# freshman97/LinTransUNet

Hardware: AMD Instinct MI355X
Metric: 128^3 CT patches/sec (fwd+bwd) (higher is better)
Workload: dtype bf16; 1 GPU; MaskTransUnet train step (fwd + 5-level loss + bwd), 128^3 single-channel patches, 2 per GPU, dropout 0.3, random-init weights; global_batch=2, parallelism=dp1, side_stream_concurrent=True, allreduce=none (1 rank)

## Files before the change

include/ltu_hip.h:

```cpp
#ifndef LTU_HIP_H
#define LTU_HIP_H

#include <stdint.h>

#ifdef __cplusplus
extern "C" {
#endif

typedef void* ltu_stream_t;

enum { LTU_F32 = 0, LTU_BF16 = 1 };
enum { LTU_OK = 0, LTU_E_DTYPE = -1, LTU_E_SHAPE = -2, LTU_E_ALIGN = -3, LTU_E_ARG = -4,
       LTU_E_COMM = -100  };
enum { LTU_ACT_NONE = 0, LTU_ACT_LRELU = 1 };

int ltu_version(void);
int ltu_build_flags(void);
int ltu_config_set(const char* name, int value, int clear);
int ltu_selftest_group_reduce(const float* x, float* sum, float* mx, int n, int G, ltu_stream_t s);
#ifdef LTU_EXPERIMENTS
int ltu_selftest_last_arriver(const float* x, float* part, float* out, unsigned* counter, float* sink, int nwg, int n,
                              int rows_per_chunk, int skew, int mode, ltu_stream_t s);
#endif

// ... 107 lines not shown

int ltu_head_softmax_fwd(const void* z, float* p, long long M, int C, int CP, int dtype, ltu_stream_t s);
int ltu_head_softmax_bwd(const float* dp, const float* p, void* dz, long long M, int C, int CP, int dtype, ltu_stream_t s);
int ltu_final_softmax_fwd(const void* z, float* p, int B, int h, int w, int D, int C, int CP, int dtype, ltu_stream_t s);
int ltu_final_softmax_bwd(const float* dp, const float* p, void* dz, int B, int h, int w, int D, int C, int CP, int dtype,
                          ltu_stream_t s);
int ltu_onehot_argmax(const float* p, float* o, long long M, int C, ltu_stream_t s);

int ltu_gate_fwd(const void* u1, const void* u2, const float* sums1, const float* sums2, const float* psi_w,
                 const float* psi_b, const void* skip, float* a_out, void* out, int B, long long S, int C, int dtype,
                 ltu_stream_t s);
int ltu_gate_bwd(const void* dout, const void* u1, const void* u2, const float* sums1, const float* sums2,
                 const float* psi_w, const void* skip, const float* a_in, void* dskip, float* ds_ws, float* dpsi_w,
                 float* dpsi_b, float* bs1, float* bs2, float* ws, long long ws_floats, void* du1, void* du2, int B, long long S, int C,
                 int dtype, ltu_stream_t s);

int ltu_dwconv_fwd(const void* x, const float* w, const float* bias, void* y, int B, int H, int W, int D, int C, float p,
                   uint64_t seed, const uint64_t* step, int dtype, ltu_stream_t s);
long long ltu_dwconv_bwd_ws_floats(int B, int H, int W, int D, int C, int dtype);
int ltu_dwconv_bwd(const void* dy, const void* dy2, const void* x, const float* w, void* dx, float* dw, float* db, float* ws,
                   long long ws_floats, int B, int H, int W, int D, int C, float p, uint64_t seed, const uint64_t* step, int dtype, ltu_stream_t s);

int ltu_roi_plan_size(int B, int H, int W, int roi_size, long long* n_int, long long* n_float, long long* n_hist);
int ltu_roi_plan(const float* prob, int B, int H, int W, int D, int C, int roi_size, float thr, float* box, int* plan_i,
                 float* plan_f, int* hist, ltu_stream_t s);
int ltu_roi_resample(const void* in, void* out, int* plan_i, float* plan_f, int which, int adjoint, int B, int H, int W,
                     int D, int C, int roi_size, int dtype, ltu_stream_t s);

int ltu_trilinear_up(const void* in, const void* in2, void* out, int adjoint, int B, int H, int W, int D, int C, int sd, int dtype,
                     ltu_stream_t s);
// ... 111 lines not shown
```

lintransunet_amd/_lib.py:

```python
import ctypes
import os
from ctypes import c_float, c_int, c_longlong, c_uint64, c_void_p

_HERE = os.path.dirname(os.path.abspath(__file__))
LIB_PATH = os.path.join(_HERE, os.environ.get('LTU_LIB', 'libltu_hip.so'))

P, I, L, F, U = c_void_p, c_int, c_longlong, c_float, c_uint64


class ReduceJob(ctypes.Structure):
    _fields_ = [('part', c_void_p), ('nsplit', c_int), ('n', c_int), ('k', c_int), ('nseg', c_int),
                ('out', c_void_p * 3), ('outb', c_void_p * 3), ('mode', c_int)]


class WgradJob(ctypes.Structure):
    _fields_ = [('grad', c_void_p), ('a', c_void_p), ('dw', c_void_p * 3), ('db', c_void_p * 3),
                ('ldg', c_int), ('lda', c_int), ('nw', c_int), ('M', c_int), ('N', c_int), ('K', c_int)]


WGRAD_GROUP_MAX = 32
CROP_ORIENT_MAX = 64
BLEND_ITEMS_MAX = 32
U8, I16 = 2, 3

# ... 76 lines not shown
    'ltu_instnorm_stats': [P, P, P, L, I, L, I, I, P],
    'ltu_instnorm_apply': [P, P, P, P, I, L, I, I, F, F, U, P, I, P],
    'ltu_instnorm_fwd': [P, P, P, L, P, P, I, L, I, I, F, F, U, P, I, P],
    'ltu_instnorm_bwd': [P, P, P, P, P, P, P, L, P, I, L, I, I, F, F, U, P, I, P],
    'ltu_layernorm_fwd': [P, P, P, P, P, P, L, I, F, F, U, P, I, P],
    'ltu_layernorm_bwd': [P, P, P, P, P, P, P, P, P, P, L, P, L, I, F, U, P, I, P],
    'ltu_gelu_dropout_fwd': [P, P, L, F, U, P, I, P],
    'ltu_gelu_dropout_bwd': [P, P, P, L, F, U, P, I, P],
    'ltu_head_softmax_fwd': [P, P, L, I, I, I, P],
    'ltu_head_softmax_bwd': [P, P, P, L, I, I, I, P],
    'ltu_final_softmax_fwd': [P, P, I, I, I, I, I, I, I, P],
    'ltu_final_softmax_bwd': [P, P, P, I, I, I, I, I, I, I, P],
    'ltu_onehot_argmax': [P, P, L, I, P],
    'ltu_gate_fwd': [P, P, P, P, P, P, P, P, P, I, L, I, I, P],
    'ltu_gate_bwd': [P, P, P, P, P, P, P, P, P, P, P, P, P, P, P, L, P, P, I, L, I, I, P],
    'ltu_dwconv_fwd': [P, P, P, P, I, I, I, I, I, F, U, P, I, P],
    'ltu_dwconv_bwd_ws_floats': [I, I, I, I, I, I],
    'ltu_dwconv_bwd': [P, P, P, P, P, P, P, P, L, I, I, I, I, I, F, U, P, I, P],
    'ltu_roi_plan_size': [I, I, I, I, P, P, P],
    'ltu_roi_plan': [P, I, I, I, I, I, I, F, P, P, P, P, P],
    'ltu_roi_resample': [P, P, P, P, I, I, I, I, I, I, I, I, I, P],
    'ltu_trilinear_up': [P, P, P, I, I, I, I, I, I, I, I, P],
    'ltu_trilinear_adjoint_ws_elems': [I, I, I, I, I, I],
    'ltu_trilinear_adjoint': [P, P, P, P, L, I, I, I, I, I, I, I, P],
    'ltu_loss_ws_floats': [I, L, I],
    'ltu_loss_fwd': [P, P, P, L, P, P, I, L, I, F, F, P, P, P],
    'ltu_loss_bwd': [P, P, P, P, P, I, L, I, P],
    'ltu_loss_wide_ws_floats': [I, L, I],
    'ltu_loss_wide_fwd': [P, P, P, L, P, P, I, L, I, F, F, P, P, P],
    'ltu_loss_wide_bwd': [P, P, P, P, P, I, L, I, P],
# ... 61 lines not shown
```

lintransunet_amd/csrc/pointwise.hip:

```cpp
#include "common.h"
#include "manyclass.h"

static unsigned sgrid(long long n, int per_block = 256) {
  long long blocks = (n + per_block - 1) / per_block;
  if (blocks > 8192) blocks = 8192;
  if (blocks < 1) blocks = 1;
  return (unsigned)blocks;
}
#define GRID_STRIDE(i, n) \
  for (long long i = (long long)blockIdx.x * blockDim.x + threadIdx.x; i < (n); i += (long long)gridDim.x * blockDim.x)

template <typename T>
__global__ void window_embed_kernel(const float* __restrict__ x, T* __restrict__ y, int B, int H, int W, int D) {
  const int h2 = H / 2, w2 = W / 2;
  const long long n = (long long)B * h2 * w2 * D;
  GRID_STRIDE(i, n) {
    const int d = (int)(i % D);
    long long t = i / D;
    const int w = (int)(t % w2);
    t /= w2;
    const int h = (int)(t % h2);
    const int b = (int)(t / h2);
    const float* xb = x + (((long long)b * H + 2 * h) * W + 2 * w) * D + d;
    float4 v = make_float4(xb[0], xb[D], xb[(long long)W * D], xb[(long long)W * D + D]);
// ... 389 lines not shown
}
extern "C" int ltu_onehot_argmax(const float* p, float* o, long long M, int C, ltu_stream_t s) {
  hipLaunchKernelGGL(onehot_argmax_kernel, dim3(sgrid(M)), dim3(256), 0, (hipStream_t)s, p, o, M, C);
  return ltu_check_launch();
}

#define IN_EPS 1e-5f
__device__ __forceinline__ void in_stat2(const float* sums, float invS, float& mean, float& rstd) {
  const float m1 = sums[1] * invS;
  const float var = fmaxf(sums[2] * invS - m1 * m1, 0.f);
  mean = sums[0] + m1;
  rstd = rsqrtf(var + IN_EPS);
}

template <typename T, int G>
__global__ void gate_fwd_kernel(const T* __restrict__ u1, const T* __restrict__ u2, const float* __restrict__ sums1,
                                const float* __restrict__ sums2, const float* __restrict__ psi_w, const float* __restrict__ psi_b,
                                const T* __restrict__ skip, float* __restrict__ a_out, T* __restrict__ out, int B, long long S) {
  const int C = G * 4;
  const int gl = threadIdx.x % G;
  const long long rows = (long long)B * S;
  const float invS = 1.f / (float)S;
  const float4 pw = *reinterpret_cast<const float4*>(psi_w + gl * 4);
  const float pb = psi_b[0];
  const long long rpb = blockDim.x / G;
  for (long long r0 = (long long)blockIdx.x * rpb; r0 < rows; r0 += (long long)gridDim.x * rpb) {
    const long long row = r0 + threadIdx.x / G;
    const bool ok = row < rows;
    float part = 0.f;
    float4 sk = make_float4(0.f, 0.f, 0.f, 0.f);
    if (ok) {
// ... 8 lines not shown
        in_stat2(sums2 + ((long long)b * C + gl * 4 + k) * 3, invS, m2, r2);
        const float r = fmaxf((f4at(a, k) - m1) * r1 + (f4at(c, k) - m2) * r2, 0.f);
        part += r * f4at(pw, k);
      }
    }
    const float sdot = group_sum<G>(part) + pb;
    const float av = 1.f / (1.f + expf(-sdot));
    if (ok) {
      if (gl == 0) a_out[row] = av;
      Vec4<T>::store(out + row * C + gl * 4, make_float4(sk.x * av, sk.y * av, sk.z * av, sk.w * av));
    }
  }
}

template <typename T, int G>
__global__ void gate_bwd_reduce_kernel(const T* __restrict__ dout, const T* __restrict__ u1, const T* __restrict__ u2,
                                       const float* __restrict__ sums1, const float* __restrict__ sums2,
                                       const float* __restrict__ psi_w, const T* __restrict__ skip, const float* __restrict__ a_in,
                                       T* __restrict__ dskip, float* __restrict__ ds_out, float* __restrict__ dpsi_w,
                                       float* __restrict__ dpsi_b, float* __restrict__ bs1, float* __restrict__ bs2,
                                       float* __restrict__ ws, int B, long long S, int rows_per_block) {
  extern __shared__ float red[];
  const int C = G * 4;
  const int gl = threadIdx.x % G, rg = threadIdx.x / G, nrg = blockDim.x / G;
  const int b = blockIdx.y;
  const float invS = 1.f / (float)S;
  const float4 pw = *reinterpret_cast<const float4*>(psi_w + gl * 4);
  float m1[4], r1[4], m2[4], r2[4];
#pragma unroll
  for (int k = 0; k < 4; ++k) {
// ... 14 lines not shown
    const bool ok = sv < s1;
    const long long row = (long long)b * S + sv;
    float4 g = make_float4(0.f, 0.f, 0.f, 0.f), sk = g, a = g, c = g;
    float av = 0.f;
    if (ok) {
      const long long e = row * C + gl * 4;
      g = Vec4<T>::load(dout + e);
      sk = Vec4<T>::load(skip + e);
      a = Vec4<T>::load(u1 + e);
      c = Vec4<T>::load(u2 + e);
      av = a_in[row];
    }
    const float da = group_sum<G>(g.x * sk.x + g.y * sk.y + g.z * sk.z + g.w * sk.w);
    const float ds = da * av * (1.f - av);
    if (ok) {
      Vec4<T>::store(dskip + row * C + gl * 4, make_float4(g.x * av, g.y * av, g.z * av, g.w * av));
      if (gl == 0) { ds_out[row] = ds; accb += ds; }
#pragma unroll
      for (int k = 0; k < 4; ++k) {
        const float h1 = (f4at(a, k) - m1[k]) * r1[k], h2 = (f4at(c, k) - m2[k]) * r2[k];
        const float r = fmaxf(h1 + h2, 0.f);
        const float dr = r > 0.f ? ds * f4at(pw, k) : 0.f;
        acc[k][0] += ds * r;
        acc[k][1] += dr;
        acc[k][2] += dr * h1;
        acc[k][3] += dr * h2;
      }
    }
  }
#pragma unroll
  for (int k = 0; k < 4; ++k) {
// ... 34 lines not shown
  }
  red[zq][el] = a0 + a1;
  __syncthreads();
  if (zq != 0 || i >= n) return;
  float v = 0.f;
#pragma unroll
  for (int q = 0; q < 32; ++q) v += red[q][el];
  const int c = i / 5, which = i % 5;
  if (which == 0) atomicAdd(dpsi_w + c, v);
  else if (which == 1) { bs1[((long long)b * C + c) * 2] += v; bs2[((long long)b * C + c) * 2] += v; }
  else if (which == 2) bs1[((long long)b * C + c) * 2 + 1] += v;
  else if (which == 3) bs2[((long long)b * C + c) * 2 + 1] += v;
  else if (c == 0) atomicAdd(dpsi_b, v);
}

template <typename T, int G>
__global__ void __launch_bounds__(256) gate_bwd_apply_kernel(const T* __restrict__ u1, const T* __restrict__ u2, const float* __restrict__ sums1,
                                      const float* __restrict__ sums2, const float* __restrict__ psi_w,
                                      const float* __restrict__ ds_in, const float* __restrict__ bs1, const float* __restrict__ bs2,
                                      T* __restrict__ du1, T* __restrict__ du2, int B, long long S) {
  constexpr int C = G * 4;
  const int b = blockIdx.y;
  const int gl = threadIdx.x % G;
  const float invS = 1.f / (float)S;
  const float4 pw = *reinterpret_cast<const float4*>(psi_w + gl * 4);
  float m1[4], r1[4], m2[4], r2[4], a1[4], b1[4], a2[4], b2[4];
#pragma unroll
  for (int k = 0; k < 4; ++k) {
    const long long bc = (long long)b * C + gl * 4 + k;
    in_stat2(sums1 + bc * 3, invS, m1[k], r1[k]);
// ... 23 lines not shown
  do {                                                        \
    if ((C) == 8) { constexpr int G = 2; __VA_ARGS__ }        \
    else if ((C) == 16) { constexpr int G = 4; __VA_ARGS__ }  \
    else if ((C) == 32) { constexpr int G = 8; __VA_ARGS__ }  \
    else if ((C) == 64) { constexpr int G = 16; __VA_ARGS__ } \
    else if ((C) == 128) { constexpr int G = 32; __VA_ARGS__ } \
    else if ((C) == 256) { constexpr int G = 64; __VA_ARGS__ } \
    else return LTU_E_SHAPE;                                  \
  } while (0)

extern "C" int ltu_gate_fwd(const void* u1, const void* u2, const float* sums1, const float* sums2, const float* psi_w,
                            const float* psi_b, const void* skip, float* a_out, void* out, int B, long long S, int C, int dtype,
                            ltu_stream_t s) {
  LTU_DISPATCH_T(dtype, {
    GATE_DISPATCH_G(C, {
      const long long rows = (long long)B * S;
      hipLaunchKernelGGL((gate_fwd_kernel<T, G>), dim3(sgrid(rows, 256 / G)), dim3(256), 0, (hipStream_t)s, (const T*)u1,
                         (const T*)u2, sums1, sums2, psi_w, psi_b, (const T*)skip, a_out, (T*)out, B, S);
    });
  });
  return ltu_check_launch();
}

extern "C" int ltu_gate_bwd(const void* dout, const void* u1, const void* u2, const float* sums1, const float* sums2,
                            const float* psi_w, const void* skip, const float* a_in, void* dskip, float* ds_ws, float* dpsi_w,
                            float* dpsi_b, float* bs1, float* bs2, float* ws, long long ws_floats, void* du1, void* du2, int B, long long S,
                            int C, int dtype, ltu_stream_t s) {
  if (ws != nullptr && ws_floats < ltu_norm_ws_floats()) return LTU_E_ARG;
  LTU_DISPATCH_T(dtype, {
    GATE_DISPATCH_G(C, {
      const int nrg = 256 / G;
      long long cap = (1 << 20) / (C * 5);
      if (cap > 2048) cap = 2048;
      long long want = cap / (B > 0 ? B : 1);
      if (want < 1) want = 1;
      long long rows = (S + want - 1) / want;
      if (rows < nrg) rows = nrg;
      rows = (rows + nrg - 1) / nrg * nrg;
      const size_t lds = (size_t)nrg * C * 5 * sizeof(float);
      hipLaunchKernelGGL((gate_bwd_reduce_kernel<T, G>), dim3(cdiv(S, rows), B), dim3(256), lds, (hipStream_t)s, (const T*)dout,
                         (const T*)u1, (const T*)u2, sums1, sums2, psi_w, (const T*)skip, a_in, (T*)dskip, ds_ws, dpsi_w, dpsi_b,
                         bs1, bs2, ws, B, S, (int)rows);
      if (ws != nullptr)
        hipLaunchKernelGGL(gate_fold_kernel, dim3(cdiv(C * 5, 32), B), dim3(1024), 0, (hipStream_t)s, ws, (int)cdiv(S, rows), C,
                           dpsi_w, dpsi_b, bs1, bs2);
      long long ablocks = (S * G + 255) / 256;
      const long long acap = 4096 / (B > 0 ? B : 1) > 1 ? 4096 / (B > 0 ? B : 1) : 1;
      if (ablocks > acap) ablocks = acap;
      hipLaunchKernelGGL((gate_bwd_apply_kernel<T, G>), dim3((unsigned)ablocks, B), dim3(256), 0, (hipStream_t)s,
                         (const T*)u1, (const T*)u2, sums1, sums2, psi_w, ds_ws, bs1, bs2, (T*)du1, (T*)du2, B, S);
    });
  });
  return ltu_check_launch();
}


#define DWH_VOX 360
#define DWH_PD 11
#define DWH_ROWS (36 * DWH_PD)
#define DWH_RUN 4
template <typename T>
__device__ __forceinline__ uint4 add16(uint4 a, uint4 b);
template <>
__device__ __forceinline__ uint4 add16<float>(uint4 a, uint4 b) {
  return make_uint4(__float_as_uint(__uint_as_float(a.x) + __uint_as_float(b.x)), __float_as_uint(__uint_as_float(a.y) + __uint_as_float(b.y)),
                    __float_as_uint(__uint_as_float(a.z) + __uint_as_float(b.z)), __float_as_uint(__uint_as_float(a.w) + __uint_as_float(b.w)));
}
template <>
// ... 305 lines not shown
```

lintransunet_amd/ops.py:

```python
import contextlib
import ctypes
import threading

import torch

from . import _lib

F32, BF16 = 0, 1
ACT_NONE, ACT_LRELU = 0, 1
LRELU_SLOPE = 0.01
_c_void_p = ctypes.c_void_p


def _dt(t):
    if t.dtype == torch.float32:
        return F32
    if t.dtype == torch.bfloat16:
        return BF16
    raise TypeError(f'unsupported activation dtype {t.dtype}')


def _p(t):
    return 0 if t is None else t.data_ptr()

# ... 1361 lines not shown
class _Gate(torch.autograd.Function):

    @staticmethod
    def forward(ctx, skip, up, wx, bx, wg, bg, pw, pb, px, pg):
        lc = ctx.lc = current()
        _chk(skip, 'skip'); _chk(up, 'up')
        B, C = skip.shape[0], skip.shape[-1]
        Cg = up.shape[-1]
        M = skip.numel() // C
        S = M // B
        dev, dt = skip.device, _dt(skip)
        u1 = torch.empty((M, C), device=dev, dtype=skip.dtype)
        u2 = torch.empty((M, C), device=dev, dtype=skip.dtype)
        wxo = px.w[0] if px is not None else _w_operand(wx, skip.dtype)
        wgo = pg.w[0] if pg is not None else _w_operand(wg, skip.dtype)
        _lib.call('ltu_linear_fwd', _p(skip), C, _ptr_array([wxo]), 1, _ptr_array([bx]), _p(u1), C, M, C, C, 0, dt, _s())
        _lib.call('ltu_linear_fwd', _p(up), Cg, _ptr_array([wgo]), 1, _ptr_array([bg]), _p(u2), C, M, C, Cg, 0, dt, _s())
        s1 = lc.scratch_zeros((B, C, 3), dev)
        s2 = lc.scratch_zeros((B, C, 3), dev)
        _lib.call('ltu_instnorm_stats', _p(u1), _p(s1), _p(lc.norm_ws(dev)), _n(lc.norm_ws(dev)), B, S, C, dt, _s())
        _lib.call('ltu_instnorm_stats', _p(u2), _p(s2), _p(lc.norm_ws(dev)), _n(lc.norm_ws(dev)), B, S, C, dt, _s())
        a = torch.empty(M, device=dev, dtype=torch.float32)
        out = torch.empty_like(skip)
        _lib.call('ltu_gate_fwd', _p(u1), _p(u2), _p(s1), _p(s2), _p(pw), _p(pb), _p(skip), _p(a), _p(out), B, S, C, dt, _s())
        ctx.save_for_backward(skip, up, u1, u2, s1, s2, a)
        ctx.params = (wx, bx, wg, bg, pw, pb)
        ctx.prep = (px, pg)
        return out

    @staticmethod
    def backward(ctx, g):
        lc = ctx.lc
        skip, up, u1, u2, s1, s2, a = ctx.saved_tensors
        wx, bx, wg, bg, pw, pb = ctx.params
        px, pg = ctx.prep
        g = g.contiguous()
        B, C = skip.shape[0], skip.shape[-1]
        Cg = up.shape[-1]
        M = skip.numel() // C
        S = M // B
        dev, dt = skip.device, _dt(skip)
        dskip = torch.empty_like(skip)
        ds = torch.empty(M, device=dev, dtype=torch.float32)
        dpw, fpw = _grad_buf(pw)
        dpb, fpb = _grad_buf(pb)
        bs1 = lc.scratch_zeros((B, C, 2), dev)
        bs2 = lc.scratch_zeros((B, C, 2), dev)
        du1 = torch.empty_like(u1)
        du2 = torch.empty_like(u2)
        _lib.call('ltu_gate_bwd', _p(g), _p(u1), _p(u2), _p(s1), _p(s2), _p(pw), _p(skip), _p(a), _p(dskip), _p(ds), _p(dpw),
                  _p(dpb), _p(bs1), _p(bs2), _p(lc.norm_ws(dev)), _n(lc.norm_ws(dev)), _p(du1), _p(du2), B, S, C, dt, _s())
        wxt = px.wt if px is not None else _w_transposed([wx], C, C, skip.dtype)
        wgt = pg.wt if pg is not None else _w_transposed([wg], C, Cg, skip.dtype)
        dup = torch.empty_like(up)
        _lib.call('ltu_linear_fwd', _p(du1), C, _ptr_array([wxt]), 1, _ptr_array([None]), _p(dskip), C, M, C, C, 1, dt, _s())
        _lib.call('ltu_linear_fwd', _p(du2), C, _ptr_array([wgt]), 1, _ptr_array([None]), _p(dup), Cg, M, Cg, C, 0, dt, _s())
        dwx, f1 = _grad_buf(wx)
        dbx, f2 = _grad_buf(bx)
        dwg, f3 = _grad_buf(wg)
        dbg, f4 = _grad_buf(bg)
        def launch(keep):
            w1, w2 = _wgrad_ws(M, C, C, skip), _wgrad_ws(M, C, Cg, skip)
            keep.extend((w1, w2))
            _lib.call('ltu_linear_wgrad', _p(du1), C, _p(skip), C, _ptr_array([dwx]), _ptr_array([dbx]), 1, M, C, C, _p(w1), _n(w1), 0, dt, _s())
            _lib.call('ltu_linear_wgrad', _p(du2), C, _p(up), Cg, _ptr_array([dwg]), _ptr_array([dbg]), 1, M, C, Cg, _p(w2), _n(w2), 0, dt, _s())
        if f1 and f2 and f3 and f4:
            lc.wq_push(launch, (du1, du2, skip, up), 'gate')
        else:
            launch([])
        return (dskip, dup, _grad_done(wx, dwx, f1), _grad_done(bx, dbx, f2), _grad_done(wg, dwg, f3), _grad_done(bg, dbg, f4),
                _grad_done(pw, dpw, fpw), _grad_done(pb, dpb, fpb), None, None)
# ... 110 lines not shown
```

Baseline: 164.0 patches/s.

## Fuse attention-gate projections with instnorm stats and fuse gate backward data path

Adds a forward kernel that computes both gate 1x1 projections with MFMA and accumulates per-channel shifted instance-norm statistics in the same pass, followed by a small fold kernel. This replaces two linear launches plus two stats passes that reread u1/u2. In backward, the elementwise gate gradient is fused with the transposed-weight matmuls that produce dskip and dup, so du1/du2 are not reread. The fused path only covers bf16 with C of 16 or 32 and adds shifted-sum numerics that differ slightly from the old stats path.

```diff
diff --git a/include/ltu_hip.h b/include/ltu_hip.h
--- a/include/ltu_hip.h
+++ b/include/ltu_hip.h
@@ -145,6 +145,14 @@
                  const float* psi_w, const void* skip, const float* a_in, void* dskip, float* ds_ws, float* dpsi_w,
                  float* dpsi_b, float* bs1, float* bs2, float* ws, long long ws_floats, void* du1, void* du2, int B, long long S, int C,
                  int dtype, ltu_stream_t s);
+int ltu_gate_fused_ok(int B, long long S, int C, int Cg, int dtype);
+int ltu_gate_proj_fwd(const void* skip, const void* up, const void* wx, const float* bx, const void* wg, const float* bg, void* u1,
+                      void* u2, float* sums1, float* sums2, float* parts, long long parts_floats, int B, long long S, int C, int dtype,
+                      ltu_stream_t s);
+int ltu_gate_bwd_fused(const void* dout, const void* u1, const void* u2, const float* sums1, const float* sums2,
+                       const float* psi_w, const void* skip, const float* a_in, const void* wxt, const void* wgt, void* dskip,
+                       void* dup, float* ds_ws, float* dpsi_w, float* dpsi_b, float* bs1, float* bs2, float* parts,
+                       long long parts_floats, void* du1, void* du2, int B, long long S, int C, int dtype, ltu_stream_t s);
 
 int ltu_dwconv_fwd(const void* x, const float* w, const float* bias, void* y, int B, int H, int W, int D, int C, float p,
                    uint64_t seed, const uint64_t* step, int dtype, ltu_stream_t s);
diff --git a/lintransunet_amd/_lib.py b/lintransunet_amd/_lib.py
--- a/lintransunet_amd/_lib.py
+++ b/lintransunet_amd/_lib.py
@@ -114,6 +114,9 @@
     'ltu_onehot_argmax': [P, P, L, I, P],
     'ltu_gate_fwd': [P, P, P, P, P, P, P, P, P, I, L, I, I, P],
     'ltu_gate_bwd': [P, P, P, P, P, P, P, P, P, P, P, P, P, P, P, L, P, P, I, L, I, I, P],
+    'ltu_gate_fused_ok': [I, L, I, I, I],
+    'ltu_gate_proj_fwd': [P, P, P, P, P, P, P, P, P, P, P, L, I, L, I, I, P],
+    'ltu_gate_bwd_fused': [P, P, P, P, P, P, P, P, P, P, P, P, P, P, P, P, P, P, L, P, P, I, L, I, I, P],
     'ltu_dwconv_fwd': [P, P, P, P, I, I, I, I, I, F, U, P, I, P],
     'ltu_dwconv_bwd_ws_floats': [I, I, I, I, I, I],
     'ltu_dwconv_bwd': [P, P, P, P, P, P, P, P, L, I, I, I, I, I, F, U, P, I, P],
diff --git a/lintransunet_amd/csrc/gate_fused.hip b/lintransunet_amd/csrc/gate_fused.hip
--- /dev/null
+++ b/lintransunet_amd/csrc/gate_fused.hip
@@ -0,0 +1,366 @@
+#include "common.h"
+
+#define IN_EPS 1e-5f
+__device__ __forceinline__ float gf_rounded(float x) {
+  asm volatile("" : "+v"(x));
+  return x;
+}
+__device__ __forceinline__ void gf_in_stat2(const float* sums, float invS, float& mean, float& rstd) {
+  const float m1 = gf_rounded(sums[1] * invS);
+  const float var = fmaxf(gf_rounded(sums[2] * invS) - gf_rounded(m1 * m1), 0.f);
+  mean = __builtin_fmaf(invS, sums[1], sums[0]);
+  rstd = rsqrtf(var + IN_EPS);
+}
+
+template <int KS, int NT>
+__device__ __forceinline__ void gf_load_w(const uint16_t* __restrict__ w, int N, int li, int lh, bf16x8 (&wf)[NT][KS]) {
+#pragma unroll
+  for (int j = 0; j < NT; ++j)
+#pragma unroll
+    for (int ks = 0; ks < KS; ++ks) {
+      const int n = j * 32 + li;
+      const uint4 v = *reinterpret_cast<const uint4*>(w + (long long)(n < N ? n : 0) * (16 * KS) + ks * 16 + lh * 8);
+      wf[j][ks] = __builtin_bit_cast(bf16x8, n < N ? v : make_uint4(0u, 0u, 0u, 0u));
+    }
+}
+
+template <int KS>
+__device__ __forceinline__ f32x16 gf_mfma(const bf16x8 (&wf)[KS], const uint4 (&x)[KS]) {
+  f32x16 acc;
+#pragma unroll
+  for (int r = 0; r < 16; ++r) acc[r] = 0.f;
+#pragma unroll
+  for (int ks = 0; ks < KS; ++ks) acc = __builtin_amdgcn_mfma_f32_32x32x16_bf16(wf[ks], __builtin_bit_cast(bf16x8, x[ks]), acc, 0, 0, 0);
+  return acc;
+}
+
+__device__ __forceinline__ uint4 gf_quad_swap(const f32x16& acc, const float4 (&bv)[4], int q) {
+  const int r0 = 2 * q, r1 = 2 * q + 1;
+  float p0x = __uint_as_float(pack_bf16x2(acc[4 * r0] + bv[r0].x, acc[4 * r0 + 1] + bv[r0].y));
+  float p0y = __uint_as_float(pack_bf16x2(acc[4 * r0 + 2] + bv[r0].z, acc[4 * r0 + 3] + bv[r0].w));
+  float p1x = __uint_as_float(pack_bf16x2(acc[4 * r1] + bv[r1].x, acc[4 * r1 + 1] + bv[r1].y));
+  float p1y = __uint_as_float(pack_bf16x2(acc[4 * r1 + 2] + bv[r1].z, acc[4 * r1 + 3] + bv[r1].w));
+  permlane32_swap(p1x, p0x);
+  permlane32_swap(p1y, p0y);
+  return make_uint4(__float_as_uint(p1x), __float_as_uint(p1y), __float_as_uint(p0x), __float_as_uint(p0y));
+}
+
+__device__ __forceinline__ void gf_unpack8(const uint4& v, float (&f)[8]) {
+  const uint32_t w[4] = {v.x, v.y, v.z, v.w};
+#pragma unroll
+  for (int i = 0; i < 4; ++i) { f[2 * i] = __uint_as_float(w[i] << 16); f[2 * i + 1] = __uint_as_float(w[i] & 0xffff0000u); }
+}
+
+struct GateProjArgs {
+  const uint16_t *skip, *up, *wx, *wg;
+  const float *bx, *bg;
+  uint16_t *u1, *u2;
+  float* parts;
+  long long S;
+};
+
+template <int C>
+__global__ void __launch_bounds__(256, 2) gate_proj_stats_kernel(const GateProjArgs a) {
+  constexpr int K1 = C / 16, K2 = C / 8, Q = C / 16;
+  __shared__ float red[4][4 * C];
+  const int lane = threadIdx.x & 63, li = lane & 31, lh = lane >> 5, wid = threadIdx.x >> 6;
+  const int b = blockIdx.y;
+  const long long ntile = a.S / 32, nwave = (long long)gridDim.x * 4;
+  const uint16_t* xs = a.skip + (long long)b * a.S * C;
+  const uint16_t* xu = a.up + (long long)b * a.S * (2 * C);
+  uint16_t* y1 = a.u1 + (long long)b * a.S * C;
+  uint16_t* y2 = a.u2 + (long long)b * a.S * C;
+  bf16x8 w1[1][K1], w2[1][K2];
+  gf_load_w<K1, 1>(a.wx, C, li, lh, w1);
+  gf_load_w<K2, 1>(a.wg, C, li, lh, w2);
+  float4 b1[4], b2[4];
+#pragma unroll
+  for (int rr = 0; rr < 4; ++rr) {
+    const int n = 8 * rr + 4 * lh;
+    b1[rr] = (a.bx != nullptr && n < C) ? *reinterpret_cast<const float4*>(a.bx + n) : make_float4(0.f, 0.f, 0.f, 0.f);
+    b2[rr] = (a.bg != nullptr && n < C) ? *reinterpret_cast<const float4*>(a.bg + n) : make_float4(0.f, 0.f, 0.f, 0.f);
+  }
+  auto fetch = [&](long long tile, uint4 (&s)[K1], uint4 (&u)[K2]) {
+    const long long row = tile * 32 + li;
+    const uint16_t* ps = xs + row * C + lh * 8;
+    const uint16_t* pu = xu + row * (2 * C) + lh * 8;
+#pragma unroll
+    for (int ks = 0; ks < K1; ++ks) s[ks] = *reinterpret_cast<const uint4*>(ps + ks * 16);
+#pragma unroll
+    for (int ks = 0; ks < K2; ++ks) u[ks] = *reinterpret_cast<const uint4*>(pu + ks * 16);
+  };
+  uint4 sc[K1], uc[K2];
+  long long tile = (long long)blockIdx.x * 4 + wid;
+  fetch(0, sc, uc);
+  uint4 sh1[Q], sh2[Q];
+  {
+    const f32x16 acc1 = gf_mfma<K1>(w1[0], sc), acc2 = gf_mfma<K2>(w2[0], uc);
+    if (tile < ntile) fetch(tile, sc, uc);
+#pragma unroll
+    for (int q = 0; q < Q; ++q) {
+      const uint4 v1 = gf_quad_swap(acc1, b1, q), v2 = gf_quad_swap(acc2, b2, q);
+      const uint32_t e1[4] = {v1.x, v1.y, v1.z, v1.w}, e2[4] = {v2.x, v2.y, v2.z, v2.w};
+      uint32_t* o1 = &sh1[q].x;
+      uint32_t* o2 = &sh2[q].x;
+#pragma unroll
+      for (int e = 0; e < 4; ++e) {
+        const uint32_t lo1 = __builtin_amdgcn_readlane(e1[e], 0), hi1 = __builtin_amdgcn_readlane(e1[e], 32);
+        const uint32_t lo2 = __builtin_amdgcn_readlane(e2[e], 0), hi2 = __builtin_amdgcn_readlane(e2[e], 32);
+        o1[e] = lh ? hi1 : lo1;
+        o2[e] = lh ? hi2 : lo2;
+      }
+    }
+  }
+  float s1a[Q][8], s1b[Q][8], s2a[Q][8], s2b[Q][8];
+#pragma unroll
+  for (int q = 0; q < Q; ++q)
+#pragma unroll
+    for (int e = 0; e < 8; ++e) { s1a[q][e] = 0.f; s1b[q][e] = 0.f; s2a[q][e] = 0.f; s2b[q][e] = 0.f; }
+  for (; tile < ntile; tile += nwave) {
+    const f32x16 acc1 = gf_mfma<K1>(w1[0], sc), acc2 = gf_mfma<K2>(w2[0], uc);
+    if (tile + nwave < ntile) fetch(tile + nwave, sc, uc);
+    const long long e0 = (tile * 32 + li) * C + (lh ? 0 : 8);
+#pragma unroll
+    for (int q = 0; q < Q; ++q) {
+      const uint4 v1 = gf_quad_swap(acc1, b1, q), v2 = gf_quad_swap(acc2, b2, q);
+      *reinterpret_cast<uint4*>(y1 + e0 + 16 * q) = v1;
+      *reinterpret_cast<uint4*>(y2 + e0 + 16 * q) = v2;
+      float f1[8], f2[8], h1[8], h2[8];
+      gf_unpack8(v1, f1);
+      gf_unpack8(v2, f2);
+      gf_unpack8(sh1[q], h1);
+      gf_unpack8(sh2[q], h2);
+#pragma unroll
+      for (int e = 0; e < 8; ++e) {
+        const float t1 = f1[e] - h1[e], t2 = f2[e] - h2[e];
+        s1a[q][e] += t1; s1b[q][e] += t1 * t1;
+        s2a[q][e] += t2; s2b[q][e] += t2 * t2;
+      }
+    }
+  }
+#pragma unroll
+  for (int q = 0; q < Q; ++q)
+#pragma unroll
+    for (int e = 0; e < 8; ++e) {
+      const float r1a = group_sum<32>(s1a[q][e]), r1b = group_sum<32>(s1b[q][e]);
+      const float r2a = group_sum<32>(s2a[q][e]), r2b = group_sum<32>(s2b[q][e]);
+      if (li == 0) {
+        const int c = 16 * q + (lh ? 0 : 8) + e;
+        red[wid][2 * c] = r1a; red[wid][2 * c + 1] = r1b;
+        red[wid][2 * C + 2 * c] = r2a; red[wid][2 * C + 2 * c + 1] = r2b;
+      }
+    }
+  __syncthreads();
+  if (threadIdx.x < 4 * C) {
+    const int i = threadIdx.x;
+    a.parts[((long long)b * gridDim.x + blockIdx.x) * (4 * C) + i] = (red[0][i] + red[1][i]) + (red[2][i] + red[3][i]);
+  }
+}
+
+template <int NB>
+__global__ void __launch_bounds__(1024) gate_stats_fold_kernel(const float* __restrict__ parts, int nparts, int C, const uint16_t* __restrict__ u1,
+                                                               const uint16_t* __restrict__ u2, long long S, float* __restrict__ sums1,
+                                                               float* __restrict__ sums2) {
+  __shared__ float red[32][33];
+  const int n = 4 * C;
+  const int el = threadIdx.x & 31, zq = threadIdx.x >> 5;
+  const int i = blockIdx.x * 32 + el, b = blockIdx.y;
+  float acc = 0.f;
+  if (i < n) {
+    const float* p = parts + (long long)b * nparts * n + i;
+    for (int z0 = zq; z0 < nparts; z0 += 32 * NB) {
+      float v[NB];
+#pragma unroll
+      for (int k = 0; k < NB; ++k) {
+        const int z = z0 + 32 * k;
+        v[k] = p[(long long)(z < nparts ? z : z0) * n];
+      }
+      float a0 = 0.f, a1 = 0.f, a2 = 0.f, a3 = 0.f;
+#pragma unroll
+      for (int k = 0; k < NB; ++k) {
+        const float t = z0 + 32 * k < nparts ? v[k] : 0.f;
+        if ((k & 3) == 0) a0 += t; else if ((k & 3) == 1) a1 += t; else if ((k & 3) == 2) a2 += t; else a3 += t;
+      }
+      acc += (a0 + a1) + (a2 + a3);
+    }
+  }
+  red[zq][el] = acc;
+  __syncthreads();
+  if (zq != 0 || i >= n) return;
+  float v = 0.f;
+#pragma unroll
+  for (int q = 0; q < 32; ++q) v += red[q][el];
+  const int t = i >= 2 * C, c = (i - t * 2 * C) >> 1, which = i & 1;
+  float* s = (t ? sums2 : sums1) + ((long long)b * C + c) * 3;
+  s[1 + which] = v;
+  if (which == 0) s[0] = bf16_to_f32((t ? u2 : u1)[(long long)b * S * C + c]);
+}
+
+static long long gate_proj_nparts(int B, long long S, int C, long long cap) {
+  const long long ntile = S / 32;
+  long long np = (ntile + 31) / 32;
+  const long long most = 1024 / B > 1 ? 1024 / B : 1;
+  if (np > most) np = most;
+  const long long fit = cap / ((long long)B * 4 * C);
+  if (np > fit) np = fit;
+  return np;
+}
+
+bool gate_fused_shape_ok(int B, long long S, int C, int Cg, int dtype) {
+  return dtype == LTU_BF16 && (C == 16 || C == 32) && Cg == 2 * C && B >= 1 && B <= 65535 && S >= 32 && S % 32 == 0 &&
+         (long long)B * 4 * C <= ltu_norm_ws_floats();
+}
+
+extern "C" int ltu_gate_fused_ok(int B, long long S, int C, int Cg, int dtype) {
+  return gate_fused_shape_ok(B, S, C, Cg, dtype) && !ltu_knob("LTU_NO_GATE_FUSED", 0) ? 1 : 0;
+}
+
+extern "C" int ltu_gate_proj_fwd(const void* skip, const void* up, const void* wx, const float* bx, const void* wg, const float* bg, void* u1,
+                                 void* u2, float* sums1, float* sums2, float* parts, long long parts_floats, int B, long long S, int C,
+                                 int dtype, ltu_stream_t s) {
+  if (!gate_fused_shape_ok(B, S, C, 2 * C, dtype)) return dtype == LTU_BF16 ? LTU_E_SHAPE : LTU_E_DTYPE;
+  if (parts == nullptr) return LTU_E_ARG;
+  const long long np = gate_proj_nparts(B, S, C, ltu_norm_ws_floats());
+  if (np < 1 || parts_floats < (long long)B * np * 4 * C) return LTU_E_ARG;
+  GateProjArgs a;
+  a.skip = (const uint16_t*)skip; a.up = (const uint16_t*)up; a.wx = (const uint16_t*)wx; a.wg = (const uint16_t*)wg;
+  a.bx = bx; a.bg = bg; a.u1 = (uint16_t*)u1; a.u2 = (uint16_t*)u2; a.parts = parts; a.S = S;
+  const dim3 grid((unsigned)np, B), fgrid(cdiv(4 * C, 32), B);
+  hipStream_t st = (hipStream_t)s;
+  if (C == 16) hipLaunchKernelGGL(gate_proj_stats_kernel<16>, grid, dim3(256), 0, st, a);
+  else hipLaunchKernelGGL(gate_proj_stats_kernel<32>, grid, dim3(256), 0, st, a);
+#define GF_FOLD(NB_) \
+  hipLaunchKernelGGL(gate_stats_fold_kernel<NB_>, fgrid, dim3(1024), 0, st, parts, (int)np, C, a.u1, a.u2, S, sums1, sums2)
+  if (np <= 128) GF_FOLD(4); else if (np <= 256) GF_FOLD(8); else if (np <= 512) GF_FOLD(16); else GF_FOLD(32);
+#undef GF_FOLD
+  return ltu_check_launch();
+}
+
+struct GateBwdArgs {
+  const uint16_t *dout, *u1, *u2, *wxt, *wgt;
+  const float *sums1, *sums2, *bs1, *bs2, *psi_w, *a, *ds;
+  uint16_t *du1, *du2, *dskip, *dup;
+  long long S;
+};
+
+template <int C>
+__global__ void __launch_bounds__(256) gate_bwd_fused_kernel(const GateBwdArgs g) {
+  constexpr int KS = C / 16, NT2 = C / 16, Q = C / 16;
+  __shared__ __attribute__((aligned(16))) float cst[9][C];
+  const int lane = threadIdx.x & 63, li = lane & 31, lh = lane >> 5, wid = threadIdx.x >> 6;
+  const int b = blockIdx.y;
+  const float invS = 1.f / (float)g.S;
+  if (threadIdx.x < C) {
+    const int c = threadIdx.x;
+    const long long bc = (long long)b * C + c;
+    float m1, r1, m2, r2;
+    gf_in_stat2(g.sums1 + bc * 3, invS, m1, r1);
+    gf_in_stat2(g.sums2 + bc * 3, invS, m2, r2);
+    cst[0][c] = m1; cst[1][c] = r1; cst[2][c] = m2; cst[3][c] = r2;
+    cst[4][c] = g.bs1[bc * 2] * invS; cst[5][c] = g.bs1[bc * 2 + 1] * invS;
+    cst[6][c] = g.bs2[bc * 2] * invS; cst[7][c] = g.bs2[bc * 2 + 1] * invS;
+    cst[8][c] = g.psi_w[c];
+  }
+  bf16x8 wx[1][KS], wg[NT2][KS];
+  gf_load_w<KS, 1>(g.wxt, C, li, lh, wx);
+  gf_load_w<KS, NT2>(g.wgt, 2 * C, li, lh, wg);
+  __syncthreads();
+  const long long ntile = g.S / 32, nwave = (long long)gridDim.x * 4;
+  const long long base = (long long)b * g.S;
+  struct Tile {
+    uint4 x1[KS], x2[KS], go[Q];
+    float av, ds;
+  };
+  auto fetch = [&](long long tile, Tile& t) {
+    const long long row = base + tile * 32 + li;
+    const long long e = row * C + lh * 8, eo = row * C + (lh ? 0 : 8);
+#pragma unroll
+    for (int ks = 0; ks < KS; ++ks) {
+      t.x1[ks] = *reinterpret_cast<const uint4*>(g.u1 + e + ks * 16);
+      t.x2[ks] = *reinterpret_cast<const uint4*>(g.u2 + e + ks * 16);
+    }
+#pragma unroll
+    for (int q = 0; q < Q; ++q) t.go[q] = *reinterpret_cast<const uint4*>(g.dout + eo + q * 16);
+    t.av = g.a[row];
+    t.ds = g.ds[row];
+  };
+  const float4 zero4[4] = {make_float4(0.f, 0.f, 0.f, 0.f), make_float4(0.f, 0.f, 0.f, 0.f), make_float4(0.f, 0.f, 0.f, 0.f),
+                           make_float4(0.f, 0.f, 0.f, 0.f)};
+  Tile cur, nxt;
+  long long tile = (long long)blockIdx.x * 4 + wid;
+  if (tile >= ntile) return;
+  fetch(tile, cur);
+  for (; tile < ntile; tile += nwave) {
+    const bool more = tile + nwave < ntile;
+    if (more) fetch(tile + nwave, nxt);
+    const long long row = base + tile * 32 + li;
+    uint4 d1[KS], d2[KS];
+#pragma unroll
+    for (int ks = 0; ks < KS; ++ks) {
+      float k9[9][8];
+#pragma unroll
+      for (int kind = 0; kind < 9; ++kind) {
+        const float4 lo = *reinterpret_cast<const float4*>(&cst[kind][ks * 16 + lh * 8]);
+        const float4 hi = *reinterpret_cast<const float4*>(&cst[kind][ks * 16 + lh * 8 + 4]);
+        k9[kind][0] = lo.x; k9[kind][1] = lo.y; k9[kind][2] = lo.z; k9[kind][3] = lo.w;
+        k9[kind][4] = hi.x; k9[kind][5] = hi.y; k9[kind][6] = hi.z; k9[kind][7] = hi.w;
+      }
+      float xa[8], xc[8], o1[8], o2[8];
+      gf_unpack8(cur.x1[ks], xa);
+      gf_unpack8(cur.x2[ks], xc);
+#pragma unroll
+      for (int k = 0; k < 8; ++k) {
+        const float e1 = xa[k] - k9[0][k], e2 = xc[k] - k9[2][k];
+        const float h1 = e1 * k9[1][k], h2 = e2 * k9[3][k];
+        const float dr = __builtin_fmaf(e1, k9[1][k], h2) > 0.f ? cur.ds * k9[8][k] : 0.f;
+        o1[k] = k9[1][k] * __builtin_fmaf(-h1, k9[5][k], dr - k9[4][k]);
+        o2[k] = k9[3][k] * __builtin_fmaf(-h2, k9[7][k], dr - k9[6][k]);
+      }
+      d1[ks] = make_uint4(pack_bf16x2(o1[0], o1[1]), pack_bf16x2(o1[2], o1[3]), pack_bf16x2(o1[4], o1[5]), pack_bf16x2(o1[6], o1[7]));
+      d2[ks] = make_uint4(pack_bf16x2(o2[0], o2[1]), pack_bf16x2(o2[2], o2[3]), pack_bf16x2(o2[4], o2[5]), pack_bf16x2(o2[6], o2[7]));
+      *reinterpret_cast<uint4*>(g.du1 + row * C + ks * 16 + lh * 8) = d1[ks];
+      *reinterpret_cast<uint4*>(g.du2 + row * C + ks * 16 + lh * 8) = d2[ks];
+    }
+    const f32x16 acc1 = gf_mfma<KS>(wx[0], d1);
+#pragma unroll
+    for (int q = 0; q < Q; ++q) {
+      const uint4 v = gf_quad_swap(acc1, zero4, q);
+      const uint32_t nv[4] = {v.x, v.y, v.z, v.w};
+      float gf[8];
+      gf_unpack8(cur.go[q], gf);
+      uint32_t rv[4];
+#pragma unroll
+      for (int e = 0; e < 4; ++e) {
+        const uint32_t ov = pack_bf16x2(gf[2 * e] * cur.av, gf[2 * e + 1] * cur.av);
+        rv[e] = pack_bf16x2(__uint_as_float(nv[e] << 16) + __uint_as_float(ov << 16),
+                            __uint_as_float(nv[e] & 0xffff0000u) + __uint_as_float(ov & 0xffff0000u));
+      }
+      *reinterpret_cast<uint4*>(g.dskip + row * C + 16 * q + (lh ? 0 : 8)) = make_uint4(rv[0], rv[1], rv[2], rv[3]);
+    }
+#pragma unroll
+    for (int j = 0; j < NT2; ++j) {
+      const f32x16 acc2 = gf_mfma<KS>(wg[j], d2);
+#pragma unroll
+      for (int q = 0; q < 2; ++q)
+        *reinterpret_cast<uint4*>(g.dup + row * (2 * C) + j * 32 + 16 * q + (lh ? 0 : 8)) = gf_quad_swap(acc2, zero4, q);
+    }
+    if (more) cur = nxt;
+  }
+}
+
+int launch_gate_bwd_fused(const void* dout, const void* u1, const void* u2, const float* sums1, const float* sums2, const float* psi_w,
+                          const float* a_in, const float* ds, const float* bs1, const float* bs2, const void* wxt, const void* wgt, void* du1,
+                          void* du2, void* dskip, void* dup, int B, long long S, int C, hipStream_t st) {
+  GateBwdArgs g;
+  g.dout = (const uint16_t*)dout; g.u1 = (const uint16_t*)u1; g.u2 = (const uint16_t*)u2; g.wxt = (const uint16_t*)wxt;
+  g.wgt = (const uint16_t*)wgt; g.sums1 = sums1; g.sums2 = sums2; g.bs1 = bs1; g.bs2 = bs2; g.psi_w = psi_w; g.a = a_in; g.ds = ds;
+  g.du1 = (uint16_t*)du1; g.du2 = (uint16_t*)du2; g.dskip = (uint16_t*)dskip; g.dup = (uint16_t*)dup; g.S = S;
+  const long long ntile = S / 32;
+  long long blocks = (ntile + 15) / 16;
+  const long long most = 2048 / B > 1 ? 2048 / B : 1;
+  if (blocks > most) blocks = most;
+  const dim3 grid((unsigned)blocks, B);
+  if (C == 16) hipLaunchKernelGGL(gate_bwd_fused_kernel<16>, grid, dim3(256), 0, st, g);
+  else hipLaunchKernelGGL(gate_bwd_fused_kernel<32>, grid, dim3(256), 0, st, g);
+  return ltu_check_launch();
+}
diff --git a/lintransunet_amd/csrc/pointwise.hip b/lintransunet_amd/csrc/pointwise.hip
--- a/lintransunet_amd/csrc/pointwise.hip
+++ b/lintransunet_amd/csrc/pointwise.hip
@@ -427,7 +427,7 @@
 }
 
 template <typename T, int G>
-__global__ void gate_fwd_kernel(const T* __restrict__ u1, const T* __restrict__ u2, const float* __restrict__ sums1,
+__global__ void gate_fwd_rowstat_kernel(const T* __restrict__ u1, const T* __restrict__ u2, const float* __restrict__ sums1,
                                 const float* __restrict__ sums2, const float* __restrict__ psi_w, const float* __restrict__ psi_b,
                                 const T* __restrict__ skip, float* __restrict__ a_out, T* __restrict__ out, int B, long long S) {
   const int C = G * 4;
@@ -466,6 +466,48 @@
 }
 
 template <typename T, int G>
+__global__ void __launch_bounds__(256) gate_fwd_kernel(const T* __restrict__ u1, const T* __restrict__ u2, const float* __restrict__ sums1,
+                                const float* __restrict__ sums2, const float* __restrict__ psi_w, const float* __restrict__ psi_b,
+                                const T* __restrict__ skip, float* __restrict__ a_out, T* __restrict__ out, int B, long long S) {
+  constexpr int C = G * 4;
+  const int gl = threadIdx.x % G;
+  const int b = blockIdx.y;
+  const float invS = 1.f / (float)S;
+  const float4 pw = *reinterpret_cast<const float4*>(psi_w + gl * 4);
+  const float pb = psi_b[0];
+  float m1[4], r1[4], m2[4], r2[4];
+#pragma unroll
+  for (int k = 0; k < 4; ++k) {
+    in_stat2(sums1 + ((long long)b * C + gl * 4 + k) * 3, invS, m1[k], r1[k]);
+    in_stat2(sums2 + ((long long)b * C + gl * 4 + k) * 3, invS, m2[k], r2[k]);
+  }
+  constexpr int rpb = 256 / G;
+  for (long long r0 = (long long)blockIdx.x * rpb; r0 < S; r0 += (long long)gridDim.x * rpb) {
+    const long long sv = r0 + threadIdx.x / G;
+    const bool ok = sv < S;
+    const long long row = (long long)b * S + sv;
+    float part = 0.f;
+    float4 sk = make_float4(0.f, 0.f, 0.f, 0.f);
+    if (ok) {
+      const long long e = row * C + gl * 4;
+      const float4 a = Vec4<T>::load(u1 + e), c = Vec4<T>::load(u2 + e);
+      sk = Vec4<T>::load(skip + e);
+#pragma unroll
+      for (int k = 0; k < 4; ++k) {
+        const float r = fmaxf((f4at(a, k) - m1[k]) * r1[k] + (f4at(c, k) - m2[k]) * r2[k], 0.f);
+        part += r * f4at(pw, k);
+      }
+    }
+    const float sdot = group_sum<G>(part) + pb;
+    const float av = 1.f / (1.f + expf(-sdot));
+    if (ok) {
+      if (gl == 0) a_out[row] = av;
+      Vec4<T>::store(out + row * C + gl * 4, make_float4(sk.x * av, sk.y * av, sk.z * av, sk.w * av));
+    }
+  }
+}
+
+template <typename T, int G, bool DSKIP = true>
 __global__ void gate_bwd_reduce_kernel(const T* __restrict__ dout, const T* __restrict__ u1, const T* __restrict__ u2,
                                        const float* __restrict__ sums1, const float* __restrict__ sums2,
                                        const float* __restrict__ psi_w, const T* __restrict__ skip, const float* __restrict__ a_in,
@@ -510,7 +552,7 @@
     const float da = group_sum<G>(g.x * sk.x + g.y * sk.y + g.z * sk.z + g.w * sk.w);
     const float ds = da * av * (1.f - av);
     if (ok) {
-      Vec4<T>::store(dskip + row * C + gl * 4, make_float4(g.x * av, g.y * av, g.z * av, g.w * av));
+      if (DSKIP) Vec4<T>::store(dskip + row * C + gl * 4, make_float4(g.x * av, g.y * av, g.z * av, g.w * av));
       if (gl == 0) { ds_out[row] = ds; accb += ds; }
 #pragma unroll
       for (int k = 0; k < 4; ++k) {
@@ -575,6 +617,10 @@
   else if (c == 0) atomicAdd(dpsi_b, v);
 }
 
+static void launch_gate_fold(const float* ws, int nparts, int C, int B, float* dpsi_w, float* dpsi_b, float* bs1, float* bs2, hipStream_t st) {
+  hipLaunchKernelGGL(gate_fold_kernel, dim3(cdiv(C * 5, 32), B), dim3(1024), 0, st, ws, nparts, C, dpsi_w, dpsi_b, bs1, bs2);
+}
+
 template <typename T, int G>
 __global__ void __launch_bounds__(256) gate_bwd_apply_kernel(const T* __restrict__ u1, const T* __restrict__ u2, const float* __restrict__ sums1,
                                       const float* __restrict__ sums2, const float* __restrict__ psi_w,
@@ -628,12 +674,39 @@
                             ltu_stream_t s) {
   LTU_DISPATCH_T(dtype, {
     GATE_DISPATCH_G(C, {
-      const long long rows = (long long)B * S;
-      hipLaunchKernelGGL((gate_fwd_kernel<T, G>), dim3(sgrid(rows, 256 / G)), dim3(256), 0, (hipStream_t)s, (const T*)u1,
+      if (ltu_knob("LTU_NO_GATE_FUSED", 0)) {
+        hipLaunchKernelGGL((gate_fwd_rowstat_kernel<T, G>), dim3(sgrid((long long)B * S, 256 / G)), dim3(256), 0, (hipStream_t)s, (const T*)u1,
+                           (const T*)u2, sums1, sums2, psi_w, psi_b, (const T*)skip, a_out, (T*)out, B, S);
+        return ltu_check_launch();
+      }
+      long long blocks = (S * G + 255) / 256;
+      const long long cap = 8192 / (B > 0 ? B : 1) > 1 ? 8192 / (B > 0 ? B : 1) : 1;
+      if (blocks > cap) blocks = cap;
+      hipLaunchKernelGGL((gate_fwd_kernel<T, G>), dim3((unsigned)blocks, B), dim3(256), 0, (hipStream_t)s, (const T*)u1,
                          (const T*)u2, sums1, sums2, psi_w, psi_b, (const T*)skip, a_out, (T*)out, B, S);
     });
   });
   return ltu_check_launch();
+}
+
+template <typename T, int G, bool DSKIP>
+static void launch_gate_bwd_reduce(const void* dout, const void* u1, const void* u2, const float* sums1, const float* sums2, const float* psi_w,
+                                   const void* skip, const float* a_in, void* dskip, float* ds_ws, float* dpsi_w, float* dpsi_b, float* bs1,
+                                   float* bs2, float* ws, int B, long long S, hipStream_t st) {
+  constexpr int C = G * 4;
+  const int nrg = 256 / G;
+  long long cap = (1 << 20) / (C * 5);
+  if (cap > 2048) cap = 2048;
+  long long want = cap / (B > 0 ? B : 1);
+  if (want < 1) want = 1;
+  long long rows = (S + want - 1) / want;
+  if (rows < nrg) rows = nrg;
+  rows = (rows + nrg - 1) / nrg * nrg;
+  const size_t lds = (size_t)nrg * C * 5 * sizeof(float);
+  hipLaunchKernelGGL((gate_bwd_reduce_kernel<T, G, DSKIP>), dim3(cdiv(S, rows), B), dim3(256), lds, st, (const T*)dout, (const T*)u1,
+                     (const T*)u2, sums1, sums2, psi_w, (const T*)skip, a_in, (T*)dskip, ds_ws, dpsi_w, dpsi_b, bs1, bs2, ws, B, S,
+                     (int)rows);
+  if (ws != nullptr) launch_gate_fold(ws, (int)cdiv(S, rows), C, B, dpsi_w, dpsi_b, bs1, bs2, st);
 }
 
 extern "C" int ltu_gate_bwd(const void* dout, const void* u1, const void* u2, const float* sums1, const float* sums2,
@@ -643,21 +716,8 @@
   if (ws != nullptr && ws_floats < ltu_norm_ws_floats()) return LTU_E_ARG;
   LTU_DISPATCH_T(dtype, {
     GATE_DISPATCH_G(C, {
-      const int nrg = 256 / G;
-      long long cap = (1 << 20) / (C * 5);
-      if (cap > 2048) cap = 2048;
-      long long want = cap / (B > 0 ? B : 1);
-      if (want < 1) want = 1;
-      long long rows = (S + want - 1) / want;
-      if (rows < nrg) rows = nrg;
-      rows = (rows + nrg - 1) / nrg * nrg;
-      const size_t lds = (size_t)nrg * C * 5 * sizeof(float);
-      hipLaunchKernelGGL((gate_bwd_reduce_kernel<T, G>), dim3(cdiv(S, rows), B), dim3(256), lds, (hipStream_t)s, (const T*)dout,
-                         (const T*)u1, (const T*)u2, sums1, sums2, psi_w, (const T*)skip, a_in, (T*)dskip, ds_ws, dpsi_w, dpsi_b,
-                         bs1, bs2, ws, B, S, (int)rows);
-      if (ws != nullptr)
-        hipLaunchKernelGGL(gate_fold_kernel, dim3(cdiv(C * 5, 32), B), dim3(1024), 0, (hipStream_t)s, ws, (int)cdiv(S, rows), C,
-                           dpsi_w, dpsi_b, bs1, bs2);
+      launch_gate_bwd_reduce<T, G, true>(dout, u1, u2, sums1, sums2, psi_w, skip, a_in, dskip, ds_ws, dpsi_w, dpsi_b, bs1, bs2, ws, B, S,
+                                         (hipStream_t)s);
       long long ablocks = (S * G + 255) / 256;
       const long long acap = 4096 / (B > 0 ? B : 1) > 1 ? 4096 / (B > 0 ? B : 1) : 1;
       if (ablocks > acap) ablocks = acap;
@@ -666,6 +726,27 @@
     });
   });
   return ltu_check_launch();
+}
+
+bool gate_fused_shape_ok(int B, long long S, int C, int Cg, int dtype);
+int launch_gate_bwd_fused(const void* dout, const void* u1, const void* u2, const float* sums1, const float* sums2, const float* psi_w,
+                          const float* a_in, const float* ds, const float* bs1, const float* bs2, const void* wxt, const void* wgt, void* du1,
+                          void* du2, void* dskip, void* dup, int B, long long S, int C, hipStream_t st);
+extern "C" int ltu_gate_bwd_fused(const void* dout, const void* u1, const void* u2, const float* sums1, const float* sums2,
+                                  const float* psi_w, const void* skip, const float* a_in, const void* wxt, const void* wgt, void* dskip,
+                                  void* dup, float* ds_ws, float* dpsi_w, float* dpsi_b, float* bs1, float* bs2, float* parts,
+                                  long long parts_floats, void* du1, void* du2, int B, long long S, int C, int dtype, ltu_stream_t s) {
+  if (!gate_fused_shape_ok(B, S, C, 2 * C, dtype)) return dtype == LTU_BF16 ? LTU_E_SHAPE : LTU_E_DTYPE;
+  if (parts == nullptr || parts_floats < ltu_norm_ws_floats()) return LTU_E_ARG;
+  typedef bf16_t T;
+  if (C == 16)
+    launch_gate_bwd_reduce<T, 4, false>(dout, u1, u2, sums1, sums2, psi_w, skip, a_in, nullptr, ds_ws, dpsi_w, dpsi_b, bs1, bs2, parts, B, S,
+                                        (hipStream_t)s);
+  else
+    launch_gate_bwd_reduce<T, 8, false>(dout, u1, u2, sums1, sums2, psi_w, skip, a_in, nullptr, ds_ws, dpsi_w, dpsi_b, bs1, bs2, parts, B, S,
+                                        (hipStream_t)s);
+  return launch_gate_bwd_fused(dout, u1, u2, sums1, sums2, psi_w, a_in, ds_ws, bs1, bs2, wxt, wgt, du1, du2, dskip, dup, B, S, C,
+                               (hipStream_t)s);
 }
 
 
diff --git a/lintransunet_amd/ops.py b/lintransunet_amd/ops.py
--- a/lintransunet_amd/ops.py
+++ b/lintransunet_amd/ops.py
@@ -1399,12 +1399,17 @@
         u2 = torch.empty((M, C), device=dev, dtype=skip.dtype)
         wxo = px.w[0] if px is not None else _w_operand(wx, skip.dtype)
         wgo = pg.w[0] if pg is not None else _w_operand(wg, skip.dtype)
-        _lib.call('ltu_linear_fwd', _p(skip), C, _ptr_array([wxo]), 1, _ptr_array([bx]), _p(u1), C, M, C, C, 0, dt, _s())
-        _lib.call('ltu_linear_fwd', _p(up), Cg, _ptr_array([wgo]), 1, _ptr_array([bg]), _p(u2), C, M, C, Cg, 0, dt, _s())
         s1 = lc.scratch_zeros((B, C, 3), dev)
         s2 = lc.scratch_zeros((B, C, 3), dev)
-        _lib.call('ltu_instnorm_stats', _p(u1), _p(s1), _p(lc.norm_ws(dev)), _n(lc.norm_ws(dev)), B, S, C, dt, _s())
-        _lib.call('ltu_instnorm_stats', _p(u2), _p(s2), _p(lc.norm_ws(dev)), _n(lc.norm_ws(dev)), B, S, C, dt, _s())
+        ctx.fused = fused = bool(_lib.load().ltu_gate_fused_ok(B, S, C, Cg, dt))
+        if fused:
+            _lib.call('ltu_gate_proj_fwd', _p(skip), _p(up), _p(wxo), _p(bx), _p(wgo), _p(bg), _p(u1), _p(u2), _p(s1), _p(s2),
+                      _p(lc.norm_ws(dev)), _n(lc.norm_ws(dev)), B, S, C, dt, _s())
+        else:
+            _lib.call('ltu_linear_fwd', _p(skip), C, _ptr_array([wxo]), 1, _ptr_array([bx]), _p(u1), C, M, C, C, 0, dt, _s())
+            _lib.call('ltu_linear_fwd', _p(up), Cg, _ptr_array([wgo]), 1, _ptr_array([bg]), _p(u2), C, M, C, Cg, 0, dt, _s())
+            _lib.call('ltu_instnorm_stats', _p(u1), _p(s1), _p(lc.norm_ws(dev)), _n(lc.norm_ws(dev)), B, S, C, dt, _s())
+            _lib.call('ltu_instnorm_stats', _p(u2), _p(s2), _p(lc.norm_ws(dev)), _n(lc.norm_ws(dev)), B, S, C, dt, _s())
         a = torch.empty(M, device=dev, dtype=torch.float32)
         out = torch.empty_like(skip)
         _lib.call('ltu_gate_fwd', _p(u1), _p(u2), _p(s1), _p(s2), _p(pw), _p(pb), _p(skip), _p(a), _p(out), B, S, C, dt, _s())
@@ -1433,13 +1438,18 @@
         bs2 = lc.scratch_zeros((B, C, 2), dev)
         du1 = torch.empty_like(u1)
         du2 = torch.empty_like(u2)
-        _lib.call('ltu_gate_bwd', _p(g), _p(u1), _p(u2), _p(s1), _p(s2), _p(pw), _p(skip), _p(a), _p(dskip), _p(ds), _p(dpw),
-                  _p(dpb), _p(bs1), _p(bs2), _p(lc.norm_ws(dev)), _n(lc.norm_ws(dev)), _p(du1), _p(du2), B, S, C, dt, _s())
         wxt = px.wt if px is not None else _w_transposed([wx], C, C, skip.dtype)
         wgt = pg.wt if pg is not None else _w_transposed([wg], C, Cg, skip.dtype)
         dup = torch.empty_like(up)
-        _lib.call('ltu_linear_fwd', _p(du1), C, _ptr_array([wxt]), 1, _ptr_array([None]), _p(dskip), C, M, C, C, 1, dt, _s())
-        _lib.call('ltu_linear_fwd', _p(du2), C, _ptr_array([wgt]), 1, _ptr_array([None]), _p(dup), Cg, M, Cg, C, 0, dt, _s())
+        if ctx.fused:
+            _lib.call('ltu_gate_bwd_fused', _p(g), _p(u1), _p(u2), _p(s1), _p(s2), _p(pw), _p(skip), _p(a), _p(wxt), _p(wgt), _p(dskip),
+                      _p(dup), _p(ds), _p(dpw), _p(dpb), _p(bs1), _p(bs2), _p(lc.norm_ws(dev)), _n(lc.norm_ws(dev)), _p(du1), _p(du2),
+                      B, S, C, dt, _s())
+        else:
+            _lib.call('ltu_gate_bwd', _p(g), _p(u1), _p(u2), _p(s1), _p(s2), _p(pw), _p(skip), _p(a), _p(dskip), _p(ds), _p(dpw),
+                      _p(dpb), _p(bs1), _p(bs2), _p(lc.norm_ws(dev)), _n(lc.norm_ws(dev)), _p(du1), _p(du2), B, S, C, dt, _s())
+            _lib.call('ltu_linear_fwd', _p(du1), C, _ptr_array([wxt]), 1, _ptr_array([None]), _p(dskip), C, M, C, C, 1, dt, _s())
+            _lib.call('ltu_linear_fwd', _p(du2), C, _ptr_array([wgt]), 1, _ptr_array([None]), _p(dup), Cg, M, Cg, C, 0, dt, _s())
         dwx, f1 = _grad_buf(wx)
         dbx, f2 = _grad_buf(bx)
         dwg, f3 = _grad_buf(wg)
```

New measurement: 164.9 patches/s (median of 6 runs). No clear change (+0.5%).
